# fukangl/SMG-multimodal-grasping

Measured on AMD Instinct MI355X. Metric: affordance fwd+bwd passes/sec (16-rot 224^2 RGB-D), higher is better.
Workload: dtype f32; 1 GPU; 16 rot x 224^2 (S=640): fwd + Huber + bwd + Adam per GPU per step; reinforcement_net style 0; 17 trunk passes; fp32; leg=headline, rotations=16, input_size=640, parallelism=dp1

## Files before the change

### smg-multimodal-grasping_amd/csrc/engine.h

```cpp
#pragma once
#include <hip/hip_runtime.h>

#include <algorithm>
#include <cmath>
#include <cstdio>
#include <cstdlib>
#include <cstring>
#include <string>
#include <type_traits>
#include <vector>

#include "../../include/smg_hip.h"
#include "elem.cuh"
#include "scene.cuh"
#include "gemm.cuh"
#include "halo.cuh"
#include "ws.cuh"
#include "wsw.cuh"
#include "plan.h"

using namespace smg;

int smg_fail(int code, const std::string& msg);
static inline int fail(int code, const std::string& msg) { return smg_fail(code, msg); }
#define HIP_OK(expr)                                                                              \
    do {                                                                                          \
        hipError_t _e = (expr);                                                                   \
        if (_e != hipSuccess)                                                                     \
            return fail(-5, std::string(#expr) + ": " + hipGetErrorString(_e));                   \
    } while (0)

static const Layout& layout_for(int head_out) {
    static Layout L1 = build_layout(1);
    static Layout L3 = build_layout(3);
    return head_out == 3 ? L3 : L1;
}

using CfgP128x128 = GemmCfg<128, 128, 16, 2, 2, 1, true>;
using CfgP128x32 = GemmCfg<128, 32, 32, 4, 1, 1, true>;
using CfgP128x64 = GemmCfg<128, 64, 16, 2, 2, 1, true>;
using CfgP64x64 = GemmCfg<64, 64, 32, 2, 2, 1, true>;
using CfgP32x64 = GemmCfg<32, 64, 32, 1, 2, 2, true>;
using CfgP64x128 = GemmCfg<64, 128, 16, 2, 2, 1, true>;
using CfgP64x32 = GemmCfg<64, 32, 64, 2, 1, 2, true>;
using CfgW32x128 = GemmCfg<32, 128, 32, 1, 4, 1, false>;
using CfgW128x64 = GemmCfg<128, 64, 16, 2, 2, 1, false>;
using CfgW128x128 = GemmCfg<128, 128, 16, 2, 2, 1, false>;
using CfgW64x64 = GemmCfg<64, 64, 16, 2, 2, 1, false>;
using CfgW64x256 = GemmCfg<64, 256, 16, 2, 2, 1, false>;

template <class C, int PREC, int MUL = 2>
using MC = typename std::conditional<PREC == 0, C, GemmCfg<C::BM, C::BN, MUL * C::BK, C::WM, C::WN, C::WK, C::AT>>::type;
enum Kind {
    K_STEM = 0, K_C1, K_C3, K_TRANS, K_HEAD0, K_D3, K_W3, K_D1, K_W1, K_TW, K_TD, K_SW, K_HW0, K_HD0, K_OTHER, K_COUNT
};
static const char* kKindNames[K_COUNT] = {"stem7x7_fwd", "conv1x1_fwd", "conv3x3_fwd", "transition_fwd", "head_conv0_fwd",
                                          "conv3x3_dgrad", "conv3x3_wgrad", "conv1x1_dgrad", "conv1x1_wgrad",
                                          "transition_wgrad", "transition_dgrad", "stem_wgrad", "head_conv0_wgrad",
                                          "head_conv0_dgrad", "elementwise"};

constexpr int kGroup = GROUP_MAX;
constexpr int kRing = kGroup + 2;

constexpr int kDbRep = 8;
struct DbSeg { int64_t grad_off; int scr_off; int n; };

struct ProfRec { hipEvent_t a, b; int kind; double flops; int stage; double bytes; };

struct StatArr { int64_t off; int stride; };

struct smg_engine {
    int device = 0, S = 0, max_streams = 0, max_pairs = 0, head_out = 1;
    Plane p_img, p_stem, p_blk[4];
    int OH = 1, OW = 1;
    const Layout* L = nullptr;

    float* img4 = nullptr; float* stem = nullptr; float* X[4] = {}; float* Bt = nullptr;
    std::vector<int64_t> bt_off[4];
    unsigned char* argmax = nullptr;
    float* F = nullptr; float* H1 = nullptr;
    float* G[4] = {}; float* GS[kRing] = {}; float* D2[kRing] = {}; float* part = nullptr; int64_t part_floats = 0;
    float* DY2 = nullptr; float* D2S[kRing] = {};
    hipStream_t side = nullptr; hipEvent_t ev_gs[kRing] = {}, ev_d2[kRing] = {}, ev_side[kRing] = {}, ev_misc = nullptr, ev_end = nullptr; float* DY0 = nullptr; float* DH1 = nullptr; float* DF = nullptr;
    double* fstat = nullptr; int64_t fstat_span = 0;
    double* bstat = nullptr; int64_t bstat_span = 0;
    float* dbscr = nullptr; int db_total = 0; int db_off[4][24] = {}; int db_toff[3] = {}; struct DbSeg* d_dbseg = nullptr; int n_dbseg = 0;
    StatArr st_stem, st_X[4], st_F, st_H1; std::vector<StatArr> st_Bt[4];
    u32x4* packed_u = nullptr; int64_t packed_units = 0;
    float* packed_f = nullptr; int64_t packed_floats = 0;
    PackDesc* d_pack = nullptr; std::vector<PackDesc> h_pack[3]; std::vector<PackDesc> h_pack_head[3];
    int pack_stride = 0, bnupd_stride = 0, n_bnupd = 0;
    int64_t pk_conv0 = 0, pk_conv0_1 = 0, pk_head0 = 0, pk_hd0 = 0, pk_head1 = 0;
    std::vector<int64_t> pk_c1[4], pk_d1[4], pk_g3f[4], pk_g3d[4], pk_hf[4], pk_hd[4]; int64_t pk_t[3] = {}, pk_td[3] = {};
    int max_pack = 0;
    float* asc = nullptr; ActScaleDesc* d_asc = nullptr; int n_asc = 0;
    unsigned* gamax = nullptr; int64_t gamax_words = 0;
    float* stab = nullptr; int64_t stab_floats = 0;
    int64_t sx_tab[4] = {}, sb_tab[4][24] = {}, sf_tab = 0;
    BnUpdDesc* d_bnupd = nullptr;
    bool have_fwd = false; int f_trunk = 0, f_head = 0, f_streams = 0, f_pairs = 0;
    bool bw_phase0_done = false;
    bool f_dense_dq = false;
    int head_bwd = 0;
    bool f_stem1 = false;
    int* d_stream_image = nullptr; int* d_stream_rot = nullptr; int* d_pair_a = nullptr; int* d_pair_b = nullptr;
    int* d_seq_t = nullptr; int* d_seq_h = nullptr; int* d_user_ptr = nullptr; int* d_user_pair = nullptr; int* d_user_slot = nullptr;
    float* d_affine = nullptr;
    float* scene_val = nullptr; int* scene_idx = nullptr; int scene_tiles = 0;
    int* d_stage = nullptr; int* h_stage[2] = {}; hipEvent_t ev_stage[2] = {}; int stage_ints = 0, stage_turn = 0;
    int so_image = 0, so_rot = 0, so_pa = 0, so_pb = 0, so_seq_t = 0, so_seq_h = 0, so_uptr = 0, so_upair = 0, so_uslot = 0, so_aff = 0, so_ma = 0, so_mb = 0, so_adam = 0;
    bool capturing = false; int* h_stage_g = nullptr; hipEvent_t ev_graph = nullptr, ev_gin = nullptr; hipStream_t gstream = nullptr; struct StepGraph* step_graph = nullptr;
    int64_t workspace_bytes = 0;
    int n_cu = 256;
    int prec = 0;
    bool serialize = false;
    bool deterministic = false;
    bool generic3x3 = false, generic_c1 = false, generic_w1 = false, stem_plane_tail = false;
    float* stemv = nullptr; float* mom_part = nullptr; double* mom = nullptr; int mom_groups = 0;
    int dbg_stop = -1;
    float* dbg_gsnap = nullptr; int64_t dbg_gsnap_floats = 0;
    bool prof = false; std::vector<ProfRec> recs; std::vector<hipEvent_t> ev_pool;
    double prof_ms[5][K_COUNT] = {}; int64_t prof_n[5][K_COUNT] = {}; double prof_flops[5][K_COUNT] = {}; double prof_bytes[5][K_COUNT] = {}; int prof_stage = -1;
    int launch_rc = 0;
};

constexpr int kMomTilesPerWg = 8;
static inline int stem_mom_tiles_x(const Plane& ps) { return (ps.W + kMomT - 1) / kMomT; }
static inline int stem_mom_tiles(const Plane& ps) { return stem_mom_tiles_x(ps) * ((ps.H + kMomT - 1) / kMomT); }
static inline int stem_mom_groups(const Plane& ps) { return (stem_mom_tiles(ps) + kMomTilesPerWg - 1) / kMomTilesPerWg; }

static Plane make_plane(int H, int W) {
    Plane p; p.H = H; p.W = W; p.HW = H * W;
    const int g = p.HW >= 8192 ? 128 : 64;
    p.HWp = (p.HW + g - 1) / g * g;
    return p;
}

template <class T>
static int dev_alloc(smg_engine* e, T** out, int64_t count) {
    void* p = nullptr;
    hipError_t err = hipMalloc(&p, (size_t)count * sizeof(T));
    if (err != hipSuccess) return fail(-12, std::string("hipMalloc ") + std::to_string(count * sizeof(T)) + " B: " + hipGetErrorString(err));
    e->workspace_bytes += count * (int64_t)sizeof(T);
    *out = (T*)p;
    return 0;
}
#define ALLOC(ptr, count) do { int _r = dev_alloc(e, &(ptr), (count)); if (_r) return _r; } while (0)

static hipEvent_t prof_event(smg_engine* e) {
    if (!e->ev_pool.empty()) { hipEvent_t ev = e->ev_pool.back(); e->ev_pool.pop_back(); return ev; }
    hipEvent_t ev; (void)hipEventCreate(&ev); return ev;
}
#define ESZ(e) ((e)->prec ? 2.0 : 4.0)
struct ProfScope {
    smg_engine* e; hipStream_t st; int kind; double flops, bytes; hipEvent_t a{}, b{};
    ProfScope(smg_engine* e_, hipStream_t s, int k, double f, double by) : e(e_), st(s), kind(k), flops(f), bytes(by) {
        if (e->prof) { a = prof_event(e); b = prof_event(e); (void)hipEventRecord(a, st); }
    }
    ~ProfScope() {
        if (e->prof) { (void)hipEventRecord(b, st); e->recs.push_back({a, b, kind, flops, e->prof_stage, bytes}); }
    }
};

#define PTAG std::integral_constant<int, PREC>{}
#define PREC_DISPATCH(e, CALL)                                            \
    switch ((e)->prec) {                                                  \
        case 1: { constexpr int PREC = 1; CALL; } break;                  \
        case 2: { constexpr int PREC = 2; CALL; } break;                  \
        default: { constexpr int PREC = 0; CALL; } break;                 \
    }

namespace {
struct TraceScope {
    hipStream_t st; int kind; dim3 grid; const char* what; unsigned long long* tbuf = nullptr; size_t n_wg = 0;
    TraceScope(hipStream_t s, int k, dim3 g, bool traced, const char* w) : st(s), kind(k), grid(g), what(w) {
        static const int tr_kind = getenv("SMG_TRACE_KIND") ? atoi(getenv("SMG_TRACE_KIND")) : -1;
        static const int tr_skip = getenv("SMG_TRACE_SKIP") ? atoi(getenv("SMG_TRACE_SKIP")) : 0;
        static int tr_seen = 0;
        if (!(traced && kind == tr_kind && tr_seen++ == tr_skip)) return;
        n_wg = (size_t)grid.x * grid.y * grid.z;
        (void)hipMalloc((void**)&tbuf, n_wg * 64);
        (void)hipMemsetAsync(tbuf, 0, n_wg * 64, st);
        (void)hipMemcpyToSymbolAsync(HIP_SYMBOL(g_smg_trace), &tbuf, sizeof(tbuf), 0, hipMemcpyHostToDevice, st);
    }
    ~TraceScope() {
        if (!tbuf) return;
        unsigned long long* nul = nullptr;
        (void)hipMemcpyToSymbolAsync(HIP_SYMBOL(g_smg_trace), &nul, sizeof(nul), 0, hipMemcpyHostToDevice, st);
        std::vector<unsigned long long> h(n_wg * 8);
        (void)hipMemcpyAsync(h.data(), tbuf, n_wg * 64, hipMemcpyDeviceToHost, st);
        (void)hipStreamSynchronize(st);
        (void)hipFree(tbuf);
        double sum[4] = {0, 0, 0, 0}, life = 0, extra = 0; size_t live = 0; unsigned long long t_min = ~0ull, t_max = 0;
        for (size_t w = 0; w < n_wg; ++w) {
            const unsigned long long* r = &h[w * 8];
            if (!r[4]) continue;
            ++live;
            if (r[7]) extra += (double)(r[7] - r[1]);
            for (int k = 0; k < 4; ++k) sum[k] += (double)(r[k + 1] - r[k]);
            t_min = std::min(t_min, r[5]); t_max = std::max(t_max, r[6]);
// ... 136 lines not shown
```

### smg-multimodal-grasping_amd/csrc/engine.hip

```cpp
#include "engine.h"

static thread_local std::string g_err;
int smg_fail(int code, const std::string& msg) { g_err = msg; return code; }

static int engine_build(smg_engine* e) {
    const Layout& L = *e->L;
    const int NS = e->max_streams, NP = e->max_pairs;
    const int S = e->S;
    const int H1 = (S - 1) / 2 + 1, H2 = (H1 - 1) / 2 + 1;
    e->p_img = make_plane(S, S);
    e->p_stem = make_plane(H1, H1);
    int h = H2;
    for (int b = 0; b < 4; ++b) { e->p_blk[b] = make_plane(h, h); h /= 2; }
    e->OH = e->OW = e->p_blk[3].H - kHeadKernel + 1;
    if (e->OH < 1) return fail(-22, "input_size too small for the 20x20 value head");

    if (getenv("SMG_SERIALIZE")) e->serialize = true;
    const int cross = getenv("SMG_CROSSCHECK") ? atoi(getenv("SMG_CROSSCHECK")) : 0;
    e->generic3x3 = cross & 1; e->generic_c1 = cross & 2; e->generic_w1 = cross & 4; e->stem_plane_tail = cross & 8;

    ALLOC(e->img4, (int64_t)NS * e->p_img.HWp * 4);
    ALLOC(e->stem, (int64_t)NS * e->p_stem.HWp * 64);
    ALLOC(e->DY0, (int64_t)NS * e->p_stem.HWp * 64);
    ALLOC(e->argmax, (int64_t)NS * e->p_blk[0].HWp * 64);
    e->stemv = e->DY0;
    e->mom_groups = stem_mom_groups(e->p_stem);
    ALLOC(e->mom_part, (int64_t)NS * e->mom_groups * kMomVals);
    ALLOC(e->mom, (int64_t)NS * kMomOut);
    int64_t bt_total = 0;
    for (int b = 0; b < 4; ++b) {
        ALLOC(e->X[b], (int64_t)NS * e->p_blk[b].HWp * kBlockCtot[b]);
        ALLOC(e->G[b], (int64_t)NS * e->p_blk[b].HWp * kBlockCtot[b]);
        for (int i = 0; i < kBlockLayers[b]; ++i) {
            e->bt_off[b].push_back(bt_total);
            bt_total += (int64_t)NS * e->p_blk[b].HWp * kBottleneck;
        }
    }
    ALLOC(e->Bt, bt_total);
    for (int k = 0; k < kRing; ++k) {
        ALLOC(e->D2[k], (int64_t)NS * e->p_blk[0].HWp * kBottleneck);
        ALLOC(e->GS[k], (int64_t)NS * e->p_blk[0].HWp * kGrowth);
        ALLOC(e->D2S[k], (int64_t)NS * (e->p_blk[0].HWp / kScaleBlock));
        HIP_OK(hipEventCreateWithFlags(&e->ev_gs[k], hipEventDisableTiming));
        HIP_OK(hipEventCreateWithFlags(&e->ev_d2[k], hipEventDisableTiming));
        HIP_OK(hipEventCreateWithFlags(&e->ev_side[k], hipEventDisableTiming));
    }
    ALLOC(e->DY2, (int64_t)NS * e->p_blk[0].HWp * kBottleneck);
    e->scene_tiles = (int)(((int64_t)(S / 2) * (S / 2) + kSceneTile - 1) / kSceneTile);
    ALLOC(e->scene_val, (int64_t)kSceneMaps * e->scene_tiles);
    ALLOC(e->scene_idx, (int64_t)kSceneMaps * e->scene_tiles);
    HIP_OK(hipEventCreateWithFlags(&e->ev_misc, hipEventDisableTiming));
    HIP_OK(hipEventCreateWithFlags(&e->ev_end, hipEventDisableTiming));
    HIP_OK(hipStreamCreateWithFlags(&e->side, hipStreamNonBlocking));
    e->part_floats = (int64_t)24 << 20;
    for (int b = 0; b < 4; ++b) {
        const Plane& pl = e->p_blk[b];
        for (int ts : {halo_tile(pl), 8})
            e->part_floats = std::max(e->part_floats, w3_partial_floats(w3_tiling(pl, ts, NS, INT64_MAX).groups, NS));
    }
    ALLOC(e->part, e->part_floats);
    ALLOC(e->F, (int64_t)NP * e->p_blk[3].HWp * 2 * kFeat);
    ALLOC(e->DF, (int64_t)NP * e->p_blk[3].HWp * 2 * kFeat);
    ALLOC(e->H1, (int64_t)NP * e->p_blk[3].HWp * kHeadMid);
    ALLOC(e->DH1, (int64_t)NP * e->p_blk[3].HWp * kHeadMid);

    int64_t off = 0;
    auto carve = [&](int n, int stride) { StatArr s{off, stride}; off += (int64_t)n * stride; return s; };
    e->st_stem = carve(NS, 64);
    for (int b = 0; b < 4; ++b) e->st_X[b] = carve(NS, kBlockCtot[b]);
    for (int b = 0; b < 4; ++b)
        for (int i = 0; i < kBlockLayers[b]; ++i) e->st_Bt[b].push_back(carve(NS, kBottleneck));
    e->st_F = carve(NP, 2 * kFeat);
    e->st_H1 = carve(NP, kHeadMid);
    e->fstat_span = e->bstat_span = off;
    if (2 * off > kStatRepStride) return fail(-22, "batch too large for the statistic arenas (kStatRepStride in gemm.cuh)");
    ALLOC(e->fstat, kFStatRep > 1 ? (int64_t)kFStatRep * kStatRepStride : 2 * off);
    ALLOC(e->bstat, (int64_t)kStatRep * kStatRepStride);
    {
        int at = 0;
        for (int b = 0; b < 4; ++b)
            for (int i = 0; i < kBlockLayers[b]; ++i) { e->db_off[b][i] = at; at += 2 * (kBlockCin[b] + i * kGrowth); }
        for (int b = 0; b < 3; ++b) { e->db_toff[b] = at; at += 2 * kBlockCtot[b]; }
        e->db_total = at;
        ALLOC(e->dbscr, (int64_t)kDbRep * at);
        HIP_OK(hipMemset(e->dbscr, 0, (size_t)kDbRep * at * sizeof(float)));
        e->n_dbseg = 2 * (6 + 12 + 24 + 16 + 3);
        HIP_OK(hipMalloc((void**)&e->d_dbseg, (size_t)3 * e->n_dbseg * sizeof(DbSeg)));
        for (int t = 0; t < 3; ++t) {
            const TrunkRef& T = L.trunk[t];
            if ((int)T.layers[0].size() != kBlockLayers[0]) continue;
            std::vector<DbSeg> v;
            for (int b = 0; b < 4; ++b)
                for (int i = 0; i < kBlockLayers[b]; ++i) {
                    const DenseLayerRef& d = T.layers[b][i];
                    v.push_back(DbSeg{d.n1.b, e->db_off[b][i], d.cin});
                    v.push_back(DbSeg{d.n1.w, e->db_off[b][i] + d.cin, d.cin});
                }
            for (int b = 0; b < 3; ++b) {
                v.push_back(DbSeg{T.tnorm[b].b, e->db_toff[b], kBlockCtot[b]});
                v.push_back(DbSeg{T.tnorm[b].w, e->db_toff[b] + kBlockCtot[b], kBlockCtot[b]});
            }
            HIP_OK(hipMemcpy(e->d_dbseg + (size_t)t * e->n_dbseg, v.data(), v.size() * sizeof(DbSeg), hipMemcpyHostToDevice));
// ... 596 lines not shown
    return 0;
}

int smg_engine_set_option(smg_engine* e, const char* name, int value) {
    if (!e || !name) return fail(-22, "NULL argument");
    const std::string s(name);
    if (s == "deterministic") { e->deterministic = value != 0; return 0; }
    if (s == "head_bwd") {
        if (value < 0 || value > 2) return fail(-22, "head_bwd must be 0 (follow the mark of smg_loss_map / smg_loss_map_ce), 1 (per-element form) or 2 (dense form)");
        e->head_bwd = value; return 0;
    }
    if (s == "serialize") { e->serialize = value != 0; return 0; }
    if (s == "debug_stop") { e->dbg_stop = value; return 0; }
    return fail(-22, "unknown engine option '" + s + "'");
}

int smg_heightmap(const double* depth_img_dev, int h, int w, const double* intrinsics3x3, const double* cam_pose4x4,
                  const double* inv_homography3x3, int out_w, int out_h, double* out_dev, void* stream) {
    if (!depth_img_dev || !intrinsics3x3 || !cam_pose4x4 || !inv_homography3x3 || !out_dev || h < 1 || w < 1 || out_w < 1 || out_h < 1)
        return fail(-22, "bad heightmap arguments");
    hipPointerAttribute_t attr;
    HIP_OK(hipPointerGetAttributes(&attr, depth_img_dev));
    HIP_OK(hipSetDevice(attr.device));
    HeightmapArgs a;
    a.depth = depth_img_dev; a.h = h; a.w = w;
    a.fx = intrinsics3x3[0]; a.fy = intrinsics3x3[4]; a.cx = intrinsics3x3[2]; a.cy = intrinsics3x3[5];
    a.r20 = cam_pose4x4[8]; a.r21 = cam_pose4x4[9]; a.r22 = cam_pose4x4[10]; a.t2 = cam_pose4x4[11];
    for (int i = 0; i < 9; ++i) a.mi[i] = inv_homography3x3[i];
    a.out = out_dev; a.ow = out_w; a.oh = out_h;
    hipLaunchKernelGGL(heightmap_warp_kernel, dim3((out_w + 255) / 256, out_h), dim3(256), 0, (hipStream_t)stream, a);
    HIP_OK(hipGetLastError());
    return 0;
}

int smg_argmax(const float* values_dev, int n, int* idx_out_dev, float* val_out_dev, void* stream) {
    if (!values_dev || !idx_out_dev || !val_out_dev || n < 1) return fail(-22, "bad argmax arguments");
    hipPointerAttribute_t attr;
    HIP_OK(hipPointerGetAttributes(&attr, values_dev));
    HIP_OK(hipSetDevice(attr.device));
    hipLaunchKernelGGL(argmax_kernel, dim3(1), dim3(256), 0, (hipStream_t)stream, values_dev, n, idx_out_dev, val_out_dev);
    HIP_OK(hipGetLastError());
    return 0;
}

int smg_adam_step(float* params, const float* grads, float* m, float* v, int64_t offset, int64_t count, int step, float lr,
                  float beta1, float beta2, float eps, void* stream) {
    if (!params || !grads || !m || !v || count < 0 || step < 1) return fail(-22, "bad Adam arguments");
    const double bc1 = 1.0 - std::pow((double)beta1, step), bc2 = 1.0 - std::pow((double)beta2, step);
    const float step_size = (float)((double)lr / bc1);
    const float bc2_sqrt = (float)std::sqrt(bc2);
    if (count == 0) return 0;
    {
        hipPointerAttribute_t attr;
        HIP_OK(hipPointerGetAttributes(&attr, params));
        HIP_OK(hipSetDevice(attr.device));
    }
    int blocks = (int)((count + 255) / 256);
    if (blocks > 4096) blocks = 4096;
    hipLaunchKernelGGL(adam_kernel, dim3(blocks), dim3(256), 0, (hipStream_t)stream, params + offset, grads + offset, m + offset, v + offset,
                       count, step_size, beta1, beta2, eps, 1.0f, bc2_sqrt);
    HIP_OK(hipGetLastError());
    return 0;
}

int64_t smg_debug_read(smg_engine* e, const char* name, float* host_out, int64_t cap, void* stream) {
    if (!e || !name) return fail(-22, "NULL argument");
    const int NS = e->max_streams, NP = e->max_pairs;
    const float* src = nullptr; int64_t n = 0;
    std::string s(name);
    if (s == "img") {
        src = e->img4; n = (int64_t)NS * e->p_img.HWp * 4;
        if (e->f_stem1 && host_out) {
            if (cap < n) return fail(-22, "img: buffer too small");
            HIP_OK(hipSetDevice(e->device));
            HIP_OK(hipStreamSynchronize((hipStream_t)stream));
            std::vector<float> one((size_t)(n / 4));
            HIP_OK(hipMemcpy(one.data(), src, one.size() * sizeof(float), hipMemcpyDeviceToHost));
            for (int64_t i = 0; i < n / 4; ++i) { host_out[4 * i] = host_out[4 * i + 1] = host_out[4 * i + 2] = one[(size_t)i]; host_out[4 * i + 3] = 0.f; }
            return n;
        }
    }
    else if (s == "stem") { src = e->stem; n = (int64_t)NS * e->p_stem.HWp * 64; }
    else if (s == "dy0") { src = e->DY0; n = (int64_t)NS * e->p_stem.HWp * 64; }
    else if (s == "feat") { src = e->F; n = (int64_t)NP * e->p_blk[3].HWp * 2 * kFeat; }
    else if (s == "h1") { src = e->H1; n = (int64_t)NP * e->p_blk[3].HWp * kHeadMid; }
    else if (s == "df") { src = e->DF; n = (int64_t)NP * e->p_blk[3].HWp * 2 * kFeat; }
    else if (s == "dh1") { src = e->DH1; n = (int64_t)NP * e->p_blk[3].HWp * kHeadMid; }
    else if (s.size() == 2 && (s[0] == 'x' || s[0] == 'g') && s[1] >= '1' && s[1] <= '4') {
        const int b = s[1] - '1';
        src = s[0] == 'x' ? e->X[b] : e->G[b]; n = (int64_t)NS * e->p_blk[b].HWp * kBlockCtot[b];
    } else if (s.size() >= 4 && s.substr(0, 2) == "bt") {
        int b = 0, i = 0;
        if (std::sscanf(name, "bt%d_%d", &b, &i) != 2 || b < 1 || b > 4 || i < 1 || i > kBlockLayers[b - 1]) return fail(-22, "bad bt name");
        src = el(e, e->Bt, e->bt_off[b - 1][i - 1]); n = (int64_t)NS * e->p_blk[b - 1].HWp * kBottleneck;
    } else if (s == "gsnap") {
        src = e->dbg_gsnap; n = e->dbg_gsnap_floats;
        if (!src) return fail(-22, "gsnap: no debug_stop backward has run");
    } else if (s == "dy2") {
        src = e->DY2; n = (int64_t)NS * e->p_blk[0].HWp * kBottleneck;
    } else if (s.size() >= 5 && (s.substr(0, 3) == "gs_" || s.substr(0, 3) == "d2_")) {
        int b = 0, i = 0;
        if (std::sscanf(name + 3, "%d_%d", &b, &i) != 2 || b < 1 || b > 4 || i < 1 || i > kBlockLayers[b - 1]) return fail(-22, "bad ring buffer name");
        const int slot = ring_pos(b - 1, i - 1) % kRing;
        const Plane& pl = e->p_blk[b - 1];
        const bool gs = s[0] == 'g';
        const int64_t per_stream = (int64_t)pl.HWp * (gs ? kGrowth : kBottleneck);
        n = (int64_t)NS * per_stream;
        if (!host_out) return n;
        const int ns_out = (int)std::min<int64_t>(NS, cap / per_stream);
        n = ns_out * per_stream;
        if (e->prec != 0) return fail(-22, "ring buffer debug reads exist in precision mode 0 only");
        HIP_OK(hipSetDevice(e->device));
        HIP_OK(hipStreamSynchronize((hipStream_t)stream));
        if (gs || kSplitOp != 3) {
            HIP_OK(hipMemcpy(host_out, gs ? e->GS[slot] : e->D2[slot], n * sizeof(float), hipMemcpyDeviceToHost));
            return n;
        }
        std::vector<unsigned short> u((size_t)ns_out * per_stream * 2);
        std::vector<float> inv((size_t)NS * (pl.HWp / kScaleBlock));
        HIP_OK(hipMemcpy(u.data(), e->D2[slot], u.size() * sizeof(unsigned short), hipMemcpyDeviceToHost));
        HIP_OK(hipMemcpy(inv.data(), e->D2S[slot], inv.size() * sizeof(float), hipMemcpyDeviceToHost));
        auto h2f = [](unsigned h) -> double {
            const int ex = (h >> 10) & 31, man = h & 1023;
            const double v = ex == 0 ? std::ldexp((double)man, -24) : (ex == 31 ? (man ? NAN : INFINITY) : std::ldexp((double)(man | 1024), ex - 25));
            return (h & 0x8000u) ? -v : v;
        };
        for (int sn = 0; sn < ns_out; ++sn)
            for (int k8 = 0; k8 < kD2K8; ++k8)
                for (int p = 0; p < pl.HWp; ++p) {
                    const size_t uh = ((((size_t)sn * 2 + 0) * kD2K8 + k8) * pl.HWp + p) * 8, ul = ((((size_t)sn * 2 + 1) * kD2K8 + k8) * pl.HWp + p) * 8;
                    const double iv = inv[(size_t)sn * (pl.HWp / kScaleBlock) + p / kScaleBlock];
                    for (int j = 0; j < 8; ++j)
                        host_out[((size_t)sn * pl.HWp + p) * kBottleneck + 8 * k8 + j] = (float)((h2f(u[uh + j]) + h2f(u[ul + j])) * iv);
                }
        return n;
    } else if (s == "asc") {
        src = e->asc; n = 2 * e->n_asc;
    } else if (s.size() >= 6 && s.substr(0, 5) == "fs_bt") {
        int b = 0, i = 0;
        if (std::sscanf(name, "fs_bt%d_%d", &b, &i) != 2 || b < 1 || b > 4 || i < 1 || i > kBlockLayers[b - 1]) return fail(-22, "bad fs_bt name");
        n = (int64_t)4 * NS * kBottleneck;
        if (!host_out) return n;
        if (cap < n) return fail(-22, "fs_bt: buffer too small");
        HIP_OK(hipSetDevice(e->device));
        HIP_OK(hipStreamSynchronize((hipStream_t)stream));
        HIP_OK(hipMemcpy(host_out, fsum(e, e->st_Bt[b - 1][i - 1]), (size_t)NS * kBottleneck * sizeof(double), hipMemcpyDeviceToHost));
        HIP_OK(hipMemcpy(host_out + 2 * NS * kBottleneck, fsq(e, e->st_Bt[b - 1][i - 1]), (size_t)NS * kBottleneck * sizeof(double), hipMemcpyDeviceToHost));
        return n;
    } else return fail(-22, "unknown debug buffer");
    if (!host_out) return n;
    if (cap < n) n = cap;
    HIP_OK(hipSetDevice(e->device));
    HIP_OK(hipStreamSynchronize((hipStream_t)stream));
    const bool typed = e->prec != 0 && (s[0] == 'x' || s[0] == 'g' || s.substr(0, 2) == "bt");
    if (!typed) {
        HIP_OK(hipMemcpy(host_out, src, n * sizeof(float), hipMemcpyDeviceToHost));
        return n;
    }
    std::vector<unsigned short> raw((size_t)n);
    HIP_OK(hipMemcpy(raw.data(), src, n * sizeof(unsigned short), hipMemcpyDeviceToHost));
    const bool f16 = e->prec == 2 && s[0] != 'g';
    for (int64_t i = 0; i < n; ++i) {
        unsigned u;
        const unsigned h = raw[(size_t)i];
        if (!f16) u = h << 16;
        else {
// ... 55 lines not shown
```

### smg-multimodal-grasping_amd/csrc/forward.hip

```cpp
#include "engine.h"

int validate_batch(const smg_engine* e, const smg_batch* B) {
    const int NS = B->n_streams, NP = B->n_pairs;
    if (NS < 1 || NS > e->max_streams || NP < 1 || NP > e->max_pairs) return fail(-22, "batch exceeds engine capacity");
    if (!B->images_nchw_dev && !B->heightmaps_dev) return fail(-22, "no input images");
    for (int s = 0; s < NS; ++s)
        if (B->stream_image[s] < 0 || B->stream_image[s] >= B->n_images) return fail(-22, "stream_image out of range");
    if (B->masks_dev) {
        if (!B->heightmaps_dev || !B->stream_mask_a || !B->stream_mask_b) return fail(-22, "device masks need the heightmap input form and both index arrays");
        for (int s = 0; s < NS; ++s)
            if (B->stream_mask_a[s] >= B->n_masks || B->stream_mask_b[s] >= B->n_masks || (B->stream_mask_a[s] < 0 && B->stream_mask_b[s] >= 0))
                return fail(-22, "stream mask index out of range");
    }
    for (int j = 0; j < NP; ++j)
        if (B->pair_a[j] < 0 || B->pair_a[j] >= NS || B->pair_b[j] < 0 || B->pair_b[j] >= NS) return fail(-22, "pair index out of range");
    const int n_seq_t = B->bn_seq_trunk ? B->n_bn_seq_trunk : 0, n_seq_h = B->bn_seq_head ? B->n_bn_seq_head : 0;
    const int R = e->max_streams > e->max_pairs ? e->max_streams : e->max_pairs;
    if (n_seq_t > 4 * R + 16 || n_seq_h > 4 * R + 16) return fail(-22, "bn sequence too long");
    if (B->heightmaps_dev) {
        const int pad = (e->S - 2 * B->hm_size) / 2;
        if (pad < 0 || 2 * B->hm_size + 2 * pad != e->S) return fail(-22, "heightmap size does not match engine input_size");
    }
    return 0;
}
// ... 1 lines not shown
void fill_stage(const smg_engine* e, const smg_batch* B, int* h) {
    const int NS = B->n_streams, NP = B->n_pairs;
    const int n_seq_t = B->bn_seq_trunk ? B->n_bn_seq_trunk : 0, n_seq_h = B->bn_seq_head ? B->n_bn_seq_head : 0;
    memcpy(h + e->so_image, B->stream_image, NS * sizeof(int));
    memcpy(h + e->so_rot, B->stream_rotated, NS * sizeof(int));
    memcpy(h + e->so_aff, B->stream_affine, 6 * NS * sizeof(float));
    if (B->masks_dev) {
        memcpy(h + e->so_ma, B->stream_mask_a, NS * sizeof(int));
        memcpy(h + e->so_mb, B->stream_mask_b, NS * sizeof(int));
    }
    memcpy(h + e->so_pa, B->pair_a, NP * sizeof(int));
    memcpy(h + e->so_pb, B->pair_b, NP * sizeof(int));
    if (n_seq_t) memcpy(h + e->so_seq_t, B->bn_seq_trunk, n_seq_t * sizeof(int));
    if (n_seq_h) memcpy(h + e->so_seq_h, B->bn_seq_head, n_seq_h * sizeof(int));
    int* ptr = h + e->so_uptr; int* up = h + e->so_upair; int* us = h + e->so_uslot; int n = 0;
    ptr[0] = 0;
    for (int s = 0; s < NS; ++s) {
        for (int j = 0; j < NP; ++j) {
            if (B->pair_a[j] == s) { up[n] = j; us[n] = 0; ++n; }
            if (B->pair_b[j] == s) { up[n] = j; us[n] = 1; ++n; }
        }
        ptr[s + 1] = n;
    }
}

int do_forward(smg_engine* e, const smg_net* net, int trunk_id, int head_id, const smg_batch* B,
                      float* q_out, hipStream_t st) {
    const Layout& L = *e->L;
    const TrunkRef& T = L.trunk[trunk_id];
    const HeadRef& Hd = L.head[head_id];
    const int NS = B->n_streams, NP = B->n_pairs;
    if (int rc = validate_batch(e, B)) return rc;
    const int n_seq_t = B->bn_seq_trunk ? B->n_bn_seq_trunk : 0, n_seq_h = B->bn_seq_head ? B->n_bn_seq_head : 0;
    const int pad = B->heightmaps_dev ? (e->S - 2 * B->hm_size) / 2 : 0;

    if (e->capturing) {
        HIP_OK(hipMemcpyAsync(e->d_stage, e->h_stage_g, (size_t)e->stage_ints * sizeof(int), hipMemcpyHostToDevice, st));
    } else {
        const int turn = e->stage_turn; e->stage_turn ^= 1;
        HIP_OK(hipEventSynchronize(e->ev_stage[turn]));
        fill_stage(e, B, e->h_stage[turn]);
        HIP_OK(hipMemcpyAsync(e->d_stage, e->h_stage[turn], (size_t)e->stage_ints * sizeof(int), hipMemcpyHostToDevice, st));
        HIP_OK(hipEventRecord(e->ev_stage[turn], st));
    }
    if (kFStatRep > 1) HIP_OK(hipMemset2DAsync(e->fstat, kStatRepStride * sizeof(double), 0, 2 * e->fstat_span * sizeof(double), kFStatRep, st));
    else HIP_OK(hipMemsetAsync(e->fstat, 0, 2 * e->fstat_span * sizeof(double), st));

    {
        const unsigned n_pack = (unsigned)(e->h_pack[trunk_id].size() + e->h_pack_head[head_id].size());
        if (e->prec == 0 && kSplitOp == 3) {
            launch_kernel(e, scale_kernel, dim3(1, n_pack + (unsigned)e->n_asc), dim3(1024), 0, st, K_OTHER, 0, 0, false,
                          e->d_pack + (trunk_id * 3 + head_id) * e->pack_stride, (int)n_pack, e->d_asc + (trunk_id * 3 + head_id) * e->n_asc,
                          net->params, e->packed_u, e->asc, e->prec);
        }
        launch_kernel(e, pack_weights_kernel, dim3(64, n_pack), dim3(256), 0, st, K_OTHER, 0, 0, false,
                      e->d_pack + (trunk_id * 3 + head_id) * e->pack_stride, net->params, e->packed_u, e->packed_f, e->prec);
    }
    const float* P = net->params;

    auto bn_stat = [&](hipStream_t cs, const BnTab& t, int rows, const double* sum, const double* sq, int sstride, int c0, int C, int count) {
        BnStatArgs a;
        a.sum = sum; a.sq = sq; a.sstride = sstride; a.eps = kEps; a.inv_count = 1.0 / (double)count;
        a.mean = const_cast<float*>(t.mean); a.invstd = const_cast<float*>(t.invstd); a.ld = t.ld; a.c0 = c0; a.C = C; a.rows = rows;
        launch_kernel(e, bn_stat_kernel, dim3((rows * C + 255) / 256), dim3(256), 0, cs, K_OTHER, 0, 0, false, a);
    };
    auto trunk_chain = [&](const int s0, const int ns, hipStream_t cs, const int u_lo, const int u_hi) -> int {
        int unit = 0;
        auto on = [&]() { const bool r = unit >= u_lo && unit < u_hi; ++unit; return r; };
        auto xs = [&](int b) { return el(e, e->X[b], (int64_t)s0 * e->p_blk[b].HWp * kBlockCtot[b]); };
        auto st_off = [&](double* base, int stride) { return base + (int64_t)s0 * stride; };
        const bool stem1 = B->heightmaps_dev != nullptr;
        float* img4 = stem1 ? e->img4 + (int64_t)s0 * e->p_img.HWp : e->img4 + (int64_t)s0 * e->p_img.HWp * 4;
        float* stem = e->stem + (int64_t)s0 * e->p_stem.HWp * 64;
        const bool head_unit = on();
        if (head_unit) {
            PrepArgs a;
            a.images_nchw = B->images_nchw_dev; a.heightmaps = B->heightmaps_dev; a.hm = B->hm_size; a.pad = pad; a.S = e->S;
            a.mean = B->image_mean; a.stdv = B->image_std;
            a.stream_image = e->d_stream_image + s0; a.stream_affine = e->d_affine + 6 * s0; a.stream_rotated = e->d_stream_rot + s0;
            a.img4 = img4; a.img1 = stem1 ? img4 : nullptr; a.HWp = e->p_img.HWp;
            a.masks = B->masks_dev; a.stream_mask_a = e->d_stage + e->so_ma + s0; a.stream_mask_b = e->d_stage + e->so_mb + s0;
            launch_kernel(e, prep_rotate_kernel, dim3((e->S * e->S + 255) / 256, ns), dim3(256), 0, cs, K_OTHER, 0, 0, false, a);
        }
        if (head_unit) {
            auto run = [&](auto tag, auto ptag, auto mtag) {
                using Cfg = decltype(tag);
                constexpr int SM = decltype(mtag)::value;
                FwdConvP<Cfg, SM, decltype(ptag)::value> p{};
                p.src = img4; p.lds_ = 4; p.ps = e->p_img; p.po = e->p_stem; p.K = 0;
                p.wp = e->packed_u + (SM == F_STEM1 ? e->pk_conv0_1 : e->pk_conv0); p.K8tot = (SM == F_STEM1 ? 64 : 224) / 8; p.N = 64;
                p.dst = stem; p.ldd = 64; p.dcoff = 0;
                p.dsum = st_off(fsum(e, e->st_stem), 64); p.dsq = st_off(fsq(e, e->st_stem), 64); p.dstride = 64;
                launch_gemm(e, cs, p, dim3(ns * e->p_stem.HWp / Cfg::BM, 1), K_STEM, 2.0 * ns * e->p_stem.HW * 64 * 147,
                            4.0 * ns * ((double)e->p_img.HW * (SM == F_STEM1 ? 1 : 4) + (double)e->p_stem.HW * 64));
            };
            if (stem1) { PREC_DISPATCH(e, if (e->p_stem.HWp % 128 == 0) run(CfgP128x64{}, PTAG, std::integral_constant<int, F_STEM1>{}); else run(CfgP64x64{}, PTAG, std::integral_constant<int, F_STEM1>{})); }
            else { PREC_DISPATCH(e, if (e->p_stem.HWp % 128 == 0) run(CfgP128x64{}, PTAG, std::integral_constant<int, F_STEM>{}); else run(CfgP64x64{}, PTAG, std::integral_constant<int, F_STEM>{})); }
        }
        if (head_unit) {
            Pool0Args a;
            a.stem = stem; a.ps = e->p_stem; a.ssum = st_off(fsum(e, e->st_stem), 64); a.ssq = st_off(fsq(e, e->st_stem), 64);
            a.gamma = P + T.norm0.w; a.beta = P + T.norm0.b; a.eps = kEps;
            a.x1 = xs(0); a.ldx = kBlockCtot[0]; a.po = e->p_blk[0];
            a.dsum = st_off(fsum(e, e->st_X[0]), kBlockCtot[0]); a.dsq = st_off(fsq(e, e->st_X[0]), kBlockCtot[0]); a.dstride = kBlockCtot[0];
            a.argmax = e->argmax + (int64_t)s0 * e->p_blk[0].HWp * 64;
            a.stemv = (stem1 && e->prec == 0 && !e->stem_plane_tail) ? e->stemv + (int64_t)s0 * e->p_blk[0].HWp * 64 : nullptr;
            PREC_DISPATCH(e, launch_kernel(e, pool0_kernel<PREC>, dim3(e->p_blk[0].HWp / 64, ns), dim3(256), 0, cs, K_OTHER, 0, 0, false, a));
        }
        for (int b = 0; b < 4; ++b) {
            e->prof_stage = b;
            const Plane pl = e->p_blk[b];
            const int Ct = kBlockCtot[b];
            double* xsum = st_off(fsum(e, e->st_X[b]), Ct); double* xsq = st_off(fsq(e, e->st_X[b]), Ct);
            for (size_t i = 0; i < T.layers[b].size(); ++i) {
                if (!on()) continue;
                const DenseLayerRef& d = T.layers[b][i];
                float* bt = el(e, e->Bt, e->bt_off[b][i] + (int64_t)s0 * pl.HWp * kBottleneck);
                double* bsum = st_off(fsum(e, e->st_Bt[b][i]), kBottleneck); double* bsq = st_off(fsq(e, e->st_Bt[b][i]), kBottleneck);
                {
                    const BnTab t1 = bn_table(e, e->sx_tab[b], e->max_streams, s0, Ct, P + d.n1.w, P + d.n1.b);
                    if (i == 0) bn_stat(cs, t1, ns, xsum, xsq, Ct, 0, d.cin, pl.HW);
                    auto run_p = [&](auto tag, auto ptag) {
                        using Cfg0 = decltype(tag);
                        using Cfg = MC<Cfg0, decltype(ptag)::value, (Cfg0::BK < 32 ? 2 : 1)>;
                        FwdConvP<Cfg, F_ONE, decltype(ptag)::value> p{};
                        p.src = xs(b); p.lds_ = Ct; p.ps = pl; p.po = pl; p.K = d.cin; p.asc = asc_n1(e, b, (int)i);
                        p.bt = t1; p.fresh0 = i == 0 ? d.cin : d.cin - kGrowth; p.fsum = xsum; p.fsq = xsq; p.fstride = Ct; p.eps = kEps;
                        p.tw_mean = const_cast<float*>(t1.mean); p.tw_invstd = const_cast<float*>(t1.invstd);
                        p.wp = e->packed_u + e->pk_c1[b][i]; p.K8tot = d.cin / 8; p.N = kBottleneck;
                        p.dst = bt; p.ldd = kBottleneck; p.dcoff = 0;
                        p.dsum = bsum; p.dsq = bsq; p.dstride = kBottleneck;
                        launch_gemm(e, cs, p, dim3(ns * pl.HWp / Cfg::BM, kBottleneck / Cfg::BN), K_C1, 2.0 * ns * pl.HW * d.cin * kBottleneck,
                                    ESZ(e) * ns * pl.HW * (d.cin + kBottleneck));
                    };
                    auto run = [&](auto tag) { PREC_DISPATCH(e, run_p(tag, PTAG)); };
                    const int small_wgs = 320;
                    const int wg128 = ns * pl.HWp / 128, wg64 = ns * pl.HWp / 64 * 2;
                    if (!e->generic_c1 && e->prec == 0 && !(pl.HWp % 128 == 0 && wg128 >= small_wgs) && wg64 >= small_wgs && d.cin % 32 == 0 && pl.HWp % 64 == 0) {
                        Fwd1x1WsArgs a{};
                        a.src = xs(b); a.lds_ = Ct; a.pl = pl; a.K = d.cin;
                        a.bt = t1; a.fresh0 = i == 0 ? d.cin : d.cin - kGrowth; a.fsum = xsum; a.fsq = xsq; a.fstride = Ct; a.eps = kEps;
                        a.tw_mean = const_cast<float*>(t1.mean); a.tw_invstd = const_cast<float*>(t1.invstd);
                        a.wp = e->packed_u + e->pk_c1[b][i]; a.N = kBottleneck; a.asc = asc_n1(e, b, (int)i);
                        a.dst = bt; a.ldd = kBottleneck; a.dsum = bsum; a.dsq = bsq; a.dstride = kBottleneck;
                        using WG_ = WsGeoT<np_of(fwd_op(0))>;
                        const int nM = ns * pl.HWp / 64, nN = kBottleneck / WG_::BN;
                        a.tm = TileMap{nM, nN, 0};
                        launch_kernel(e, conv1x1_fwd_ws_kernel<0>, dim3(tile_grid(a.tm)), dim3(512), WG_::smem_bytes(d.cin), cs, K_C1,
                                      2.0 * ns * pl.HW * d.cin * kBottleneck, ESZ(e) * ns * pl.HW * (d.cin + kBottleneck), false, a);
                    } else
                    if (pl.HWp % 128 == 0 && wg128 >= small_wgs) run(CfgP128x128{});
                    else if (wg64 < small_wgs) run(CfgP32x64{});
                    else run(CfgP64x64{});
                }
                const BnTab t2 = bn_table(e, e->sb_tab[b][i], e->max_streams, s0, kBottleneck, P + d.n2.w, P + d.n2.b);
                if (e->generic3x3) bn_stat(cs, t2, ns, bsum, bsq, kBottleneck, 0, kBottleneck, pl.HW);
                if (!e->generic3x3) {
                    Halo3x3FwdArgs a;
                    a.src = bt; a.lds_ = kBottleneck; a.pl = pl; a.C = kBottleneck;
                    a.ssum = bsum; a.ssq = bsq; a.sstride = kBottleneck; a.gamma = P + d.n2.w; a.beta = P + d.n2.b; a.eps = kEps;
                    a.tw_mean = const_cast<float*>(t2.mean); a.tw_invstd = const_cast<float*>(t2.invstd);
                    a.dst = xs(b); a.ldd = Ct; a.dcoff = d.cin;
                    a.dsum = xsum; a.dsq = xsq; a.dstride = Ct;
                    a.wu = e->packed_u + e->pk_hf[b][i]; a.asc = asc_n2(e, b, (int)i);
                    const double flops = 2.0 * ns * pl.HW * 9 * kBottleneck * kGrowth, bytes = ESZ(e) * ns * pl.HW * (kBottleneck + kGrowth);
                    if (halo_tile(pl, ns) == 8) {
                        a.tiles_x = (pl.W + 7) / 8; a.n_tiles = ((pl.H + 7) / 8) * a.tiles_x; a.streams = ns;
                        PREC_DISPATCH(e, launch_kernel(e, conv3x3_halo_fwd_kernel<8, PREC, false, true>, dim3(banded_grid(a.n_tiles, ns)), dim3(512),
                                                       HaloFwdSGeo<8, PREC>::smem_bytes_ws(kBottleneck), cs, K_C3, flops, bytes, true, a));
                    } else {
                        a.tiles_x = (pl.W + 15) / 16; a.n_tiles = ((pl.H + 15) / 16) * a.tiles_x; a.streams = ns;
                        if (pl.H % 16 || pl.W % 16) {
                            PREC_DISPATCH(e, launch_kernel(e, conv3x3_halo_fwd_kernel<16, PREC, true>, dim3(banded_grid(a.n_tiles, ns)), dim3(256),
                                                           HaloFwdSGeo<16, PREC>::smem_bytes(kBottleneck), cs, K_C3, flops, bytes, true, a));
                        } else {
                            PREC_DISPATCH(e, launch_kernel(e, conv3x3_halo_fwd_kernel<16, PREC>, dim3(banded_grid(a.n_tiles, ns)), dim3(256),
                                                           HaloFwdSGeo<16, PREC>::smem_bytes(kBottleneck), cs, K_C3, flops, bytes, true, a));
                        }
                    }
                } else {
                    auto run = [&](auto tag) {
                        using Cfg = decltype(tag);
// ... 101 lines not shown
```

Measured before the change: 64.39 passes/s.

## Fuse stem conv with BN-ReLU-maxpool via stats pass and recompute

For the fp32 single-channel stem with more than four streams, the stem convolution is no longer written to a full-resolution buffer and re-read by the pool kernel. A first kernel computes only the per-channel BN statistics from the conv output. A second kernel recomputes the conv on pooled-output tiles in LDS and applies BN, ReLU, maxpool, argmax and the next-layer statistics. This trades a recomputed 7x7 conv (bf16-split MFMA) for removing the large stem activation write and read. New debug dump names and a crosscheck flag to disable the path are also added.

After: 64.66 passes/s (median of 6 runs). Within noise of the previous version (+0.4%).

```diff
diff --git a/smg-multimodal-grasping_amd/csrc/engine.h b/smg-multimodal-grasping_amd/csrc/engine.h
--- a/smg-multimodal-grasping_amd/csrc/engine.h
+++ b/smg-multimodal-grasping_amd/csrc/engine.h
@@ -12,6 +12,7 @@
 
 #include "../../include/smg_hip.h"
 #include "elem.cuh"
+#include "stem.cuh"
 #include "scene.cuh"
 #include "gemm.cuh"
 #include "halo.cuh"
@@ -115,7 +116,7 @@
     int prec = 0;
     bool serialize = false;
     bool deterministic = false;
-    bool generic3x3 = false, generic_c1 = false, generic_w1 = false, stem_plane_tail = false;
+    bool generic3x3 = false, generic_c1 = false, generic_w1 = false, stem_plane_tail = false, stem_plane_fwd = false;
     float* stemv = nullptr; float* mom_part = nullptr; double* mom = nullptr; int mom_groups = 0;
     int dbg_stop = -1;
     float* dbg_gsnap = nullptr; int64_t dbg_gsnap_floats = 0;
diff --git a/smg-multimodal-grasping_amd/csrc/engine.hip b/smg-multimodal-grasping_amd/csrc/engine.hip
--- a/smg-multimodal-grasping_amd/csrc/engine.hip
+++ b/smg-multimodal-grasping_amd/csrc/engine.hip
@@ -17,7 +17,7 @@
 
     if (getenv("SMG_SERIALIZE")) e->serialize = true;
     const int cross = getenv("SMG_CROSSCHECK") ? atoi(getenv("SMG_CROSSCHECK")) : 0;
-    e->generic3x3 = cross & 1; e->generic_c1 = cross & 2; e->generic_w1 = cross & 4; e->stem_plane_tail = cross & 8;
+    e->generic3x3 = cross & 1; e->generic_c1 = cross & 2; e->generic_w1 = cross & 4; e->stem_plane_tail = cross & 8; e->stem_plane_fwd = cross & 16;
 
     ALLOC(e->img4, (int64_t)NS * e->p_img.HWp * 4);
     ALLOC(e->stem, (int64_t)NS * e->p_stem.HWp * 64);
@@ -780,6 +780,18 @@
     }
     else if (s == "stem") { src = e->stem; n = (int64_t)NS * e->p_stem.HWp * 64; }
     else if (s == "dy0") { src = e->DY0; n = (int64_t)NS * e->p_stem.HWp * 64; }
+    else if (s == "stemv") { src = e->stemv; n = (int64_t)NS * e->p_blk[0].HWp * 64; }
+    else if (s == "argmax0") {
+        n = (int64_t)NS * e->p_blk[0].HWp * 64;
+        if (!host_out) return n;
+        if (cap < n) n = cap;
+        HIP_OK(hipSetDevice(e->device));
+        HIP_OK(hipStreamSynchronize((hipStream_t)stream));
+        std::vector<unsigned char> raw((size_t)n);
+        HIP_OK(hipMemcpy(raw.data(), e->argmax, (size_t)n, hipMemcpyDeviceToHost));
+        for (int64_t i = 0; i < n; ++i) host_out[i] = (float)raw[(size_t)i];
+        return n;
+    }
     else if (s == "feat") { src = e->F; n = (int64_t)NP * e->p_blk[3].HWp * 2 * kFeat; }
     else if (s == "h1") { src = e->H1; n = (int64_t)NP * e->p_blk[3].HWp * kHeadMid; }
     else if (s == "df") { src = e->DF; n = (int64_t)NP * e->p_blk[3].HWp * 2 * kFeat; }
diff --git a/smg-multimodal-grasping_amd/csrc/forward.hip b/smg-multimodal-grasping_amd/csrc/forward.hip
--- a/smg-multimodal-grasping_amd/csrc/forward.hip
+++ b/smg-multimodal-grasping_amd/csrc/forward.hip
@@ -107,7 +107,30 @@
             a.masks = B->masks_dev; a.stream_mask_a = e->d_stage + e->so_ma + s0; a.stream_mask_b = e->d_stage + e->so_mb + s0;
             launch_kernel(e, prep_rotate_kernel, dim3((e->S * e->S + 255) / 256, ns), dim3(256), 0, cs, K_OTHER, 0, 0, false, a);
         }
-        if (head_unit) {
+        const bool fused_head = e->prec == 0 && stem1 && B->n_streams > 4 && !e->stem_plane_fwd;
+        if (head_unit && fused_head) {
+            const double conv_flops = 2.0 * 64 * 147;
+            StemStatsArgs sa;
+            sa.img = img4; sa.pi = e->p_img; sa.ps = e->p_stem; sa.wp = e->packed_u + e->pk_conv0_1;
+            sa.dsum = st_off(fsum(e, e->st_stem), 64); sa.dsq = st_off(fsq(e, e->st_stem), 64);
+            launch_kernel(e, stem_stats_kernel, dim3((e->p_stem.HW + kStemStatBM - 1) / kStemStatBM, ns), dim3(256), stem_stats_smem(e->p_img, e->p_stem), cs,
+                          K_STEM, conv_flops * ns * e->p_stem.HW, 4.0 * ns * e->p_img.HW, false, sa);
+            StemPoolArgs a;
+            a.img = img4; a.pi = e->p_img; a.ps = e->p_stem; a.wp = sa.wp; a.ssum = sa.dsum; a.ssq = sa.dsq;
+            a.gamma = P + T.norm0.w; a.beta = P + T.norm0.b; a.eps = kEps;
+            a.x1 = xs(0); a.ldx = kBlockCtot[0]; a.po = e->p_blk[0];
+            a.dsum = st_off(fsum(e, e->st_X[0]), kBlockCtot[0]); a.dsq = st_off(fsq(e, e->st_X[0]), kBlockCtot[0]); a.dstride = kBlockCtot[0];
+            a.argmax = e->argmax + (int64_t)s0 * e->p_blk[0].HWp * 64;
+            a.stemv = e->stem_plane_tail ? nullptr : e->stemv + (int64_t)s0 * e->p_blk[0].HWp * 64;
+            a.stem = stem;
+            a.tiles_x = (e->p_blk[0].W + kSpTW - 1) / kSpTW;
+            const int tiles = a.tiles_x * ((e->p_blk[0].H + kSpTH - 1) / kSpTH);
+            const double flops = conv_flops * ns * tiles * (kSpWH * kSpWW);
+            const double bytes = 4.0 * ns * e->p_img.HW + (double)ns * e->p_blk[0].HW * 64 * (4 + 4 + 1);
+            if (e->stem_plane_tail) launch_kernel(e, stem_pool_kernel<true>, dim3(tiles, ns), dim3(256), kStemPoolSmem, cs, K_STEM, flops, bytes, false, a);
+            else launch_kernel(e, stem_pool_kernel<false>, dim3(tiles, ns), dim3(256), kStemPoolSmem, cs, K_STEM, flops, bytes, false, a);
+        }
+        if (head_unit && !fused_head) {
             auto run = [&](auto tag, auto ptag, auto mtag) {
                 using Cfg = decltype(tag);
                 constexpr int SM = decltype(mtag)::value;
@@ -122,7 +145,7 @@
             if (stem1) { PREC_DISPATCH(e, if (e->p_stem.HWp % 128 == 0) run(CfgP128x64{}, PTAG, std::integral_constant<int, F_STEM1>{}); else run(CfgP64x64{}, PTAG, std::integral_constant<int, F_STEM1>{})); }
             else { PREC_DISPATCH(e, if (e->p_stem.HWp % 128 == 0) run(CfgP128x64{}, PTAG, std::integral_constant<int, F_STEM>{}); else run(CfgP64x64{}, PTAG, std::integral_constant<int, F_STEM>{})); }
         }
-        if (head_unit) {
+        if (head_unit && !fused_head) {
             Pool0Args a;
             a.stem = stem; a.ps = e->p_stem; a.ssum = st_off(fsum(e, e->st_stem), 64); a.ssq = st_off(fsq(e, e->st_stem), 64);
             a.gamma = P + T.norm0.w; a.beta = P + T.norm0.b; a.eps = kEps;
diff --git a/smg-multimodal-grasping_amd/csrc/stem.cuh b/smg-multimodal-grasping_amd/csrc/stem.cuh
--- /dev/null
+++ b/smg-multimodal-grasping_amd/csrc/stem.cuh
@@ -0,0 +1,259 @@
+#pragma once
+#include "gemm.cuh"
+
+namespace smg {
+
+__device__ __forceinline__ void stem_load_b(const u32x4* wp, int l31, int half, u32x4 (&b)[4][2][3]) {
+#pragma unroll
+    for (int s = 0; s < 4; ++s)
+#pragma unroll
+        for (int j = 0; j < 2; ++j)
+#pragma unroll
+            for (int pc = 0; pc < 3; ++pc) b[s][j][pc] = wp[(pc * 8 + 2 * s + half) * 64 + j * 32 + l31];
+}
+
+__device__ __forceinline__ void stem_conv_tile(const float* img, const int o, const int pitch, const int half, const u32x4 (&b)[4][2][3],
+                                               f32x16 (&acc)[2]) {
+#pragma unroll
+    for (int j = 0; j < 2; ++j)
+#pragma unroll
+        for (int r = 0; r < 16; ++r) acc[j][r] = 0.f;
+#pragma unroll
+    for (int s = 0; s < 4; ++s) {
+        float v[8];
+#pragma unroll
+        for (int j = 0; j < 8; ++j) {
+            const int t0 = 16 * s + j, t1 = t0 + 8;
+            if (s < 3) v[j] = img[o + (half ? (t1 / 7) * pitch + t1 % 7 : (t0 / 7) * pitch + t0 % 7)];
+            else if (j == 0) { const float x = img[o + 6 * pitch + 6]; v[j] = half ? 0.f : x; }
+            else v[j] = 0.f;
+        }
+        const Split4 lo = split4<0>(make_float4(v[0], v[1], v[2], v[3])), hi = split4<0>(make_float4(v[4], v[5], v[6], v[7]));
+        u32x4 a[3];
+#pragma unroll
+        for (int pc = 0; pc < 3; ++pc) a[pc] = u32x4{lo.p[pc].x, lo.p[pc].y, hi.p[pc].x, hi.p[pc].y};
+#pragma unroll
+        for (int j = 0; j < 2; ++j) acc[j] = mfma_bf16(a[0], b[s][j][2], acc[j]);
+#pragma unroll
+        for (int j = 0; j < 2; ++j) acc[j] = mfma_bf16(a[2], b[s][j][0], acc[j]);
+#pragma unroll
+        for (int j = 0; j < 2; ++j) acc[j] = mfma_bf16(a[1], b[s][j][1], acc[j]);
+#pragma unroll
+        for (int j = 0; j < 2; ++j) acc[j] = mfma_bf16(a[0], b[s][j][1], acc[j]);
+#pragma unroll
+        for (int j = 0; j < 2; ++j) acc[j] = mfma_bf16(a[1], b[s][j][0], acc[j]);
+#pragma unroll
+        for (int j = 0; j < 2; ++j) acc[j] = mfma_bf16(a[0], b[s][j][0], acc[j]);
+    }
+}
+
+__device__ __forceinline__ void stem_stat_flush(double (&v)[2][2], double* red, double* dsum, double* dsq) {
+    const int t = threadIdx.x, lane = t & 63, wave = t >> 6;
+#pragma unroll
+    for (int q = 0; q < 2; ++q)
+#pragma unroll
+        for (int j = 0; j < 2; ++j) {
+            v[q][j] += __shfl_xor(v[q][j], 32);
+            if (lane < 32) red[(q * 4 + wave) * 64 + j * 32 + lane] = v[q][j];
+        }
+    __syncthreads();
+    if (t < 128) {
+        const int q = t >> 6, c = t & 63;
+        double tot = 0.0;
+#pragma unroll
+        for (int w = 0; w < 4; ++w) tot += red[(q * 4 + w) * 64 + c];
+        atomicAdd((q ? dsq : dsum) + c + fstat_rep(), tot);
+    }
+}
+
+constexpr int kStemStatBM = 512;
+struct StemStatsArgs {
+    const float* img; Plane pi, ps;
+    const u32x4* wp;
+    double* dsum; double* dsq;
+};
+__host__ __device__ inline int stem_stats_rows(int W) { return (kStemStatBM - 2) / W + 2; }
+__host__ __device__ inline int stem_stats_img_floats(int S, int W) { return ((2 * stem_stats_rows(W) + 5) * (S + 6) + 1) & ~1; }
+static inline size_t stem_stats_smem(const Plane& pi, const Plane& ps) { return (size_t)stem_stats_img_floats(pi.W, ps.W) * 4 + 2 * 4 * 64 * 8; }
+
+static __global__ __launch_bounds__(256, 2) void stem_stats_kernel(const StemStatsArgs a) {
+    extern __shared__ __attribute__((aligned(16))) float smem[];
+    const int n = blockIdx.y, t = threadIdx.x, lane = t & 63, wave = t >> 6, l31 = lane & 31, half = lane >> 5;
+    const int W = a.ps.W, HW = a.ps.HW, S = a.pi.W, pitch = S + 6;
+    const int p0 = blockIdx.x * kStemStatBM, p1 = min(p0 + kStemStatBM, HW);
+    const int y0 = p0 / W, y1 = (p1 - 1) / W;
+    const int nrow = 2 * (y1 - y0) + 7, gy0 = 2 * y0 - 3;
+    const float* src = a.img + (int64_t)n * a.pi.HWp;
+    for (int r = wave; r < nrow; r += 4) {
+        const int gy = gy0 + r;
+        const bool rin = (unsigned)gy < (unsigned)a.pi.H;
+        const float* srow = src + (rin ? gy : 0) * S;
+#pragma unroll 4
+        for (int c = lane; c < pitch; c += 64) {
+            const int gx = c - 3;
+            const bool in = rin && (unsigned)gx < (unsigned)S;
+            const float x = srow[in ? gx : 0];
+            smem[r * pitch + c] = in ? x : 0.f;
+        }
+    }
+    u32x4 b[4][2][3];
+    stem_load_b(a.wp, l31, half, b);
+    __syncthreads();
+    double v[2][2] = {{0.0, 0.0}, {0.0, 0.0}};
+    for (int rt = wave; rt < kStemStatBM / 32; rt += 4) {
+        const int ps0 = p0 + rt * 32;
+        if (ps0 >= HW) break;
+        const int p = min(ps0 + l31, HW - 1);
+        const int y = p / W, x = p - y * W;
+        f32x16 acc[2];
+        stem_conv_tile(smem, 2 * (y - y0) * pitch + 2 * x, pitch, half, b, acc);
+        if (ps0 + 32 <= HW) {
+#pragma unroll
+            for (int j = 0; j < 2; ++j) {
+                float s1 = 0.f, s2 = 0.f;
+                const float s = acc[j][0];
+#pragma unroll
+                for (int r = 0; r < 16; ++r) {
+                    float dx = acc[j][r] - s;
+                    asm volatile("" : "+v"(dx));
+                    s1 += dx;
+                    s2 = fmaf(dx, dx, s2);
+                }
+                const double sd = (double)s, s1d = (double)s1;
+                v[0][j] += s1d + 16.0 * sd;
+                v[1][j] += (double)s2 + 2.0 * sd * s1d + 16.0 * sd * sd;
+            }
+        } else {
+#pragma unroll
+            for (int j = 0; j < 2; ++j)
+#pragma unroll
+                for (int r = 0; r < 16; ++r)
+                    if (ps0 + SMG_ACC_ROW(0, 0, r, half) < HW) {
+                        const double xd = (double)acc[j][r];
+                        v[0][j] += xd;
+                        v[1][j] += xd * xd;
+                    }
+        }
+    }
+    stem_stat_flush(v, reinterpret_cast<double*>(smem + stem_stats_img_floats(S, W)), a.dsum + (int64_t)n * 64, a.dsq + (int64_t)n * 64);
+}
+
+constexpr int kSpTH = 7, kSpTW = 8, kSpWH = 2 * kSpTH + 1, kSpWW = 2 * kSpTW + 1, kSpLd = 68;
+constexpr int kSpIH = 2 * kSpWH + 5, kSpIW = 2 * kSpWW + 5, kSpIP = 40;
+static_assert(kSpWH * kSpWW <= 256 && kSpIW <= kSpIP, "eight MFMA tiles cover the window");
+constexpr int kSpWinFloats = 256 * kSpLd, kSpImgFloats = kSpIH * kSpIP;
+constexpr size_t kStemPoolSmem = (size_t)(kSpWinFloats + kSpImgFloats + 192) * 4;
+static_assert(kSpImgFloats * 4 >= 2 * 4 * 64 * 8, "the reduction scratch reuses the image tile");
+struct StemPoolArgs {
+    const float* img; Plane pi, ps;
+    const u32x4* wp;
+    const double* ssum; const double* ssq;
+    const float* gamma; const float* beta; float eps;
+    void* x1; int ldx; Plane po;
+    double* dsum; double* dsq; int dstride;
+    unsigned char* argmax; float* stemv;
+    float* stem;
+    int tiles_x;
+};
+
+template <bool PLANE>
+static __global__ __launch_bounds__(256, 2) void stem_pool_kernel(const StemPoolArgs a) {
+    using XT = act_t<0>;
+    extern __shared__ __attribute__((aligned(16))) float smem[];
+    float* win = smem;
+    float* tile = smem + kSpWinFloats;
+    float* prm = tile + kSpImgFloats;
+    const int n = blockIdx.y, t = threadIdx.x, lane = t & 63, wave = t >> 6, l31 = lane & 31, half = lane >> 5;
+    const int ty0 = (blockIdx.x / a.tiles_x) * kSpTH, tx0 = (blockIdx.x % a.tiles_x) * kSpTW;
+    const float* src = a.img + (int64_t)n * a.pi.HWp;
+    constexpr int NI = (kSpImgFloats + 255) / 256;
+    float iv[NI];
+#pragma unroll
+    for (int k = 0; k < NI; ++k) {
+        const int idx = t + 256 * k, r = idx / kSpIP, c = idx - r * kSpIP;
+        const int gy = 4 * ty0 - 5 + r, gx = 4 * tx0 - 5 + c;
+        const bool in = idx < kSpImgFloats && (unsigned)gy < (unsigned)a.pi.H && (unsigned)gx < (unsigned)a.pi.W;
+        const float x = src[in ? gy * a.pi.W + gx : 0];
+        iv[k] = in ? x : 0.f;
+    }
+    u32x4 b[4][2][3];
+    stem_load_b(a.wp, l31, half, b);
+    if (t < 64) {
+        float mean, invstd;
+        bn_moments(a.ssum, a.ssq, (int64_t)n * 64 + t, 1.0 / (double)a.ps.HW, a.eps, mean, invstd);
+        prm[t] = mean;
+        prm[64 + t] = a.gamma[t] * invstd;
+        prm[128 + t] = a.beta[t];
+    }
+#pragma unroll
+    for (int k = 0; k < NI; ++k)
+        if (t + 256 * k < kSpImgFloats) tile[t + 256 * k] = iv[k];
+    __syncthreads();
+#pragma unroll
+    for (int k = 0; k < 2; ++k) {
+        const int rt = wave + 4 * k;
+        const int m = min(rt * 32 + l31, kSpWH * kSpWW - 1);
+        const int wy = m / kSpWW, wx = m - wy * kSpWW;
+        f32x16 acc[2];
+        stem_conv_tile(tile, 2 * wy * kSpIP + 2 * wx, kSpIP, half, b, acc);
+#pragma unroll
+        for (int j = 0; j < 2; ++j)
+#pragma unroll
+            for (int r = 0; r < 16; ++r) win[(rt * 32 + SMG_ACC_ROW(0, 0, r, half)) * kSpLd + j * 32 + l31] = acc[j][r];
+    }
+    __syncthreads();
+    const int cq = t & 15, slot = t >> 4;
+    if constexpr (PLANE) {
+        for (int m = slot; m < kSpWH * kSpWW; m += 16) {
+            const int wy = m / kSpWW, wx = m - wy * kSpWW;
+            const int yy = 2 * ty0 - 1 + wy, xx = 2 * tx0 - 1 + wx;
+            if (wy >= 1 && wx >= 1 && yy < a.ps.H && xx < a.ps.W)
+                *reinterpret_cast<float4*>(a.stem + ((int64_t)n * a.ps.HWp + yy * a.ps.W + xx) * 64 + 4 * cq) = *reinterpret_cast<const float4*>(win + m * kSpLd + 4 * cq);
+        }
+    }
+    double s[4] = {0, 0, 0, 0}, ss[4] = {0, 0, 0, 0};
+#pragma unroll
+    for (int i4 = 0; i4 < (kSpTH * kSpTW + 15) / 16; ++i4) {
+        const int i = slot + 16 * i4;
+        const int py = i / kSpTW, px = i - py * kSpTW;
+        const int y = ty0 + py, x = tx0 + px;
+        if (i >= kSpTH * kSpTW || y >= a.po.H || x >= a.po.W) continue;
+        float best[4] = {-INFINITY, -INFINITY, -INFINITY, -INFINITY};
+        int bi[4] = {0, 0, 0, 0};
+        float raw[4] = {0.f, 0.f, 0.f, 0.f};
+#pragma unroll
+        for (int k = 0; k < 9; ++k) {
+            const int yy = 2 * y - 1 + k / 3, xx = 2 * x - 1 + k % 3;
+            if ((unsigned)yy >= (unsigned)a.ps.H || (unsigned)xx >= (unsigned)a.ps.W) continue;
+            const float4 r = *reinterpret_cast<const float4*>(win + ((2 * py + k / 3) * kSpWW + 2 * px + k % 3) * kSpLd + 4 * cq);
+            const float4 v = bnrelu4(r, prm + 4 * cq, 64);
+            const float vv[4] = {v.x, v.y, v.z, v.w}, rr[4] = {r.x, r.y, r.z, r.w};
+#pragma unroll
+            for (int c = 0; c < 4; ++c)
+                if (vv[c] > best[c]) { best[c] = vv[c]; bi[c] = k; raw[c] = rr[c]; }
+        }
+        const int64_t o = (int64_t)n * a.po.HWp + y * a.po.W + x;
+        stq<XT>(a.x1, o * a.ldx + 4 * cq, make_float4(best[0], best[1], best[2], best[3]));
+        *reinterpret_cast<uchar4*>(a.argmax + o * 64 + 4 * cq) = make_uchar4(bi[0], bi[1], bi[2], bi[3]);
+        if (a.stemv) *reinterpret_cast<float4*>(a.stemv + o * 64 + 4 * cq) = make_float4(raw[0], raw[1], raw[2], raw[3]);
+#pragma unroll
+        for (int c = 0; c < 4; ++c) { s[c] += (double)best[c]; ss[c] += (double)best[c] * (double)best[c]; }
+    }
+    double* red = reinterpret_cast<double*>(tile);
+#pragma unroll
+    for (int c = 0; c < 4; ++c) {
+        s[c] += __shfl_xor(s[c], 16); s[c] += __shfl_xor(s[c], 32);
+        ss[c] += __shfl_xor(ss[c], 16); ss[c] += __shfl_xor(ss[c], 32);
+        if (lane < 16) { red[(0 * 4 + wave) * 64 + 4 * cq + c] = s[c]; red[(1 * 4 + wave) * 64 + 4 * cq + c] = ss[c]; }
+    }
+    __syncthreads();
+    if (t < 128) {
+        const int q = t >> 6, c = t & 63;
+        double tot = 0.0;
+#pragma unroll
+        for (int w = 0; w < 4; ++w) tot += red[(q * 4 + w) * 64 + c];
+        atomicAdd((q ? a.dsq : a.dsum) + (int64_t)n * a.dstride + c + fstat_rep(), tot);
+    }
+}
+
+}
```
